# aanna0701/face-recognition-pytorch

Hardware: AMD Instinct MI355X
Metric: train imgs/sec IR-50-layout ResNet50 + ArcFace/PartialFC head, 112x112 (higher is better)
Workload: dtype bf16

## Files before the change

face-recognition-pytorch_amd/frhip/csrc/igemm_halo.h:

```cpp
#pragma once
#include <type_traits>
#include "igemm_nt.h"

#ifndef FRHIP_ABL
#define FRHIP_ABL 0
#endif

namespace frhip {

struct HaloGeom {
    int H, W, C;
    int M, Nout, Ktot;
    int sign;
    uint32_t a_bytes, b_bytes;
    const float* xf_scale;
    const float* xf_shift;
    void* xf_out;
    FastDiv d_hw, d_w;
};

template <typename T, int WM, int WN, int MT, int HBUFS>
struct HaloTile {
    static constexpr int WAVES = WM * WN, THREADS = 64 * WAVES;
    static constexpr int WROWS = MT * 16, BM = WM * WROWS, BN = WN * 64;
    static constexpr int BKE = NT_ROWB / (int)sizeof(T);
    static constexpr int MAXW = 56;
    static constexpr int HROWS = ((BM + 2 * MAXW + 2 + 7) / 8) * 8;
    static constexpr int ZROW = HROWS * NT_ROWB;
    static constexpr int HALO_BYTES = ZROW + NT_ROWB;
    static constexpr int WBUF_BYTES = BN * NT_ROWB;
    static constexpr int DUMP_OFF = HBUFS * HALO_BYTES;
    static constexpr int W_OFF = DUMP_OFF + 1024;
    static constexpr int WRING = 3;
    static constexpr int B_PIECES = (BN / 8 + WAVES - 1) / WAVES;
    static constexpr int ITER_PIECES = B_PIECES + (HBUFS == 2 ? 1 : 0);
    template <typename TS> static constexpr int stage_pitch() { return 64 * (int)sizeof(TS) + 16; }
    template <typename TS> static constexpr int lds_bytes() {
        constexpr int loop = W_OFF + WRING * WBUF_BYTES;
        constexpr int epi = WAVES * WROWS * stage_pitch<TS>();
        return loop > epi ? loop : epi;
    }
};

template <typename T, int WM, int WN, int MT, int HBUFS, bool XF = false>
struct HaloMainloop {
    static_assert(!XF || (HBUFS == 1 && std::is_same<T, bf16_t>::value), "operand transform: single-buffer bf16 tile only");
    typedef HaloTile<T, WM, WN, MT, HBUFS> Tile;
    typedef typename Mma<T>::Frag Frag;
    static constexpr int BM = Tile::BM, BN = Tile::BN, BKE = Tile::BKE;

    f32x4_t acc[4][MT];

    __device__ __forceinline__ void run(const HaloGeom& g, const void* __restrict__ a_ptr,
                                        const void* __restrict__ b_ptr, char* smem, int mtile, int ntile) {
        const int lane = lane_id(), wave = wave_id();
        const int wm = wave / WN, wn = wave % WN;
        const __amdgpu_buffer_rsrc_t ra = make_rsrc(a_ptr, g.a_bytes);
        const __amdgpu_buffer_rsrc_t rb = make_rsrc(b_ptr, g.b_bytes);
        const int m0 = mtile * BM;
        const int hrows = BM + 2 * g.W + 2;
        const int npieces = (hrows + 7) >> 3;
        const int p_lo = m0 - g.W - 1;
        const int sub = lane >> 3;
        const uint32_t chunk_bytes = (uint32_t)(((lane & 7) ^ sub) * 16);
        const int nchunks = g.C / BKE;

        const uint32_t row0_off = (uint32_t)((p_lo + sub) * g.C) * (uint32_t)sizeof(T) + chunk_bytes;
        auto halo_piece = [&](int hb, int piece, int c0) {
            const uint32_t off = row0_off + (uint32_t)(piece * 8 * g.C + c0) * (uint32_t)sizeof(T);
            glds16(ra, smem + hb * Tile::HALO_BYTES + piece * 1024, off);
        };
        auto xform_chunk = [&](int c0) {
            if constexpr (XF) {
                const int lc = (lane & 7) ^ sub;
                float sc[8], sh[8];
#pragma unroll
                for (int e = 0; e < 8; ++e) { sc[e] = g.xf_scale[c0 + 8 * lc + e]; sh[e] = g.xf_shift[c0 + 8 * lc + e]; }
                const bool emit = g.xf_out != nullptr && ntile == 0;
                for (int piece = wave; piece < npieces; piece += Tile::WAVES) {
                    const int p = p_lo + piece * 8 + sub;
                    if (p >= 0 && p < g.M) {
                        bf16x8_t* a = reinterpret_cast<bf16x8_t*>(smem + piece * 1024 + lane * 16);
                        bf16x8_t v = *a;
#pragma unroll
                        for (int e = 0; e < 8; ++e) { const float o = (float)v[e] * sc[e] + sh[e]; v[e] = (bf16_t)fmaxf(o, 0.f); }
                        *a = v;
                        if (emit && p >= m0 && p < m0 + BM)
                            *reinterpret_cast<bf16x8_t*>(reinterpret_cast<bf16_t*>(g.xf_out) + (size_t)p * g.C + c0 + 8 * lc) = v;
                    }
                }
                asm volatile("s_waitcnt lgkmcnt(0)" ::: "memory");
            }
        };
        uint32_t brow_off[Tile::B_PIECES];
#pragma unroll
        for (int j = 0; j < Tile::B_PIECES; ++j) {
            const int piece = wave * Tile::B_PIECES + j;
            const int n = ntile * BN + piece * 8 + sub;
            brow_off[j] = (piece * 8 < BN && n < g.Nout) ? (uint32_t)n * (uint32_t)g.Ktot * (uint32_t)sizeof(T) + chunk_bytes
                                                         : OOB_OFFSET;
        }
        auto weights = [&](int wit) {
            const int ch = wit / 9, tap = wit - ch * 9;
            const bool live = ch < nchunks;
            const uint32_t kb = (uint32_t)(tap * g.C + ch * BKE) * (uint32_t)sizeof(T);
            char* wb = smem + Tile::W_OFF + (wit % Tile::WRING) * Tile::WBUF_BYTES;
#pragma unroll
            for (int j = 0; j < Tile::B_PIECES; ++j) {
                const int piece = wave * Tile::B_PIECES + j;
                const bool in_tile = piece * 8 < BN;
                glds16(rb, in_tile ? wb + piece * 1024 : smem + Tile::DUMP_OFF,
                       (live && in_tile && brow_off[j] != OOB_OFFSET) ? brow_off[j] + kb : OOB_OFFSET);
            }
        };

        const int fi = lane & 15, fg = lane >> 4;
        static_assert(Tile::HALO_BYTES < 65536, "packed fragment offsets");
        uint32_t xa[9][(MT + 1) / 2];
        {
            const int HW = g.H * g.W;
            uint32_t tt[9];
#pragma unroll
// ... 61 lines not shown
                for (int nt = 0; nt < 4; ++nt) {
                    if constexpr (FRHIP_ABL & 2) { Frag fa = wf[SET][nt], fb = xf[SET][mt]; asm volatile("" :: "v"(fa), "v"(fb)); }
                    else Mma<T>::run(wf[SET][nt], xf[SET][mt], acc[nt][mt]);
                }
        };
        auto mfma_set_first = [&](auto set_c) {
            constexpr int SET = decltype(set_c)::value;
#pragma unroll
            for (int mt = 0; mt < MT; ++mt)
#pragma unroll
                for (int nt = 0; nt < 4; ++nt) {
                    f32x4_t z = f32x4_t{0.f, 0.f, 0.f, 0.f};
                    if constexpr (FRHIP_ABL & 2) { Frag fa = wf[SET][nt], fb = xf[SET][mt]; asm volatile("" :: "v"(fa), "v"(fb)); }
                    else Mma<T>::run(wf[SET][nt], xf[SET][mt], z);
                    acc[nt][mt] = z;
                }
        };
        auto interleave = [&]() {
            constexpr int NREAD = (4 + MT) * (int)(sizeof(Frag) / 16), NMFMA = 4 * MT * (sizeof(T) == 2 ? 1 : (sizeof(T) == 1 ? 2 : 4));
            constexpr int PER = NMFMA / NREAD > 0 ? NMFMA / NREAD : 1;
#pragma unroll
            for (int i = 0; i < NREAD; ++i) {
                __builtin_amdgcn_sched_group_barrier(0x008, PER, 0);
                __builtin_amdgcn_sched_group_barrier(0x100, 1, 0);
            }
        };
        typedef std::integral_constant<int, 0> I0;
        typedef std::integral_constant<int, 1> I1;

        if (threadIdx.x < 8 * HBUFS) {
            const int hbz = threadIdx.x >> 3;
            *reinterpret_cast<f32x4_t*>(smem + hbz * Tile::HALO_BYTES + Tile::ZROW + (threadIdx.x & 7) * 16) = f32x4_t{0.f, 0.f, 0.f, 0.f};
        }
        for (int piece = wave; piece < npieces; piece += Tile::WAVES) halo_piece(0, piece, 0);
        weights(0);
        weights(1);
        asm volatile("s_waitcnt vmcnt(0)" ::: "memory");
        xform_chunk(0);
        __syncthreads();
        load_frags(I0{}, I0{}, I0{}, I0{}, I0{});

        auto chunk_body = [&](auto hb_c, int ch) {
            constexpr int HB = decltype(hb_c)::value;
            constexpr int HBN = HBUFS == 2 ? (HB ^ 1) : 0;
            const int c0 = ch * BKE;
            const int it0 = ch * 9;
            auto tap_body = [&](auto tap_c) {
                constexpr int TAP = decltype(tap_c)::value;
                if constexpr (!(FRHIP_ABL & 8)) {
                    weights(it0 + TAP + 2);
                    if (HBUFS == 2) {
                        const int piece = TAP * Tile::WAVES + wave;
                        if (TAP < 8 && ch + 1 < nchunks && piece < npieces) halo_piece(HBN, piece, c0 + BKE);
                        else glds16(ra, smem + Tile::DUMP_OFF, OOB_OFFSET);
                    }
                }
                load_frags(I1{}, I1{}, hb_c, std::integral_constant<int, TAP % Tile::WRING>{}, tap_c);
                if (TAP == 0 && ch == 0) mfma_set_first(I0{});
                else mfma_set(I0{});
                interleave();
                if constexpr (FRHIP_ABL & 8) asm volatile("s_waitcnt vmcnt(0)" ::: "memory");
                else if constexpr (Tile::ITER_PIECES == 1) asm volatile("s_waitcnt vmcnt(1)" ::: "memory");
                else if constexpr (Tile::ITER_PIECES == 2) asm volatile("s_waitcnt vmcnt(2)" ::: "memory");
                else if constexpr (Tile::ITER_PIECES == 3) asm volatile("s_waitcnt vmcnt(3)" ::: "memory");
                else if constexpr (Tile::ITER_PIECES == 4) asm volatile("s_waitcnt vmcnt(4)" ::: "memory");
                else asm volatile("s_waitcnt vmcnt(5)" ::: "memory");
                static_assert(Tile::ITER_PIECES <= 5, "add a vmcnt case");
                if constexpr (!(FRHIP_ABL & 1)) __builtin_amdgcn_s_barrier();
                if constexpr (TAP < 8)
                    load_frags(I0{}, I0{}, hb_c, std::integral_constant<int, (TAP + 1) % Tile::WRING>{}, std::integral_constant<int, (TAP + 1) % 9>{});
                else
                    load_frags(I0{}, I0{}, std::integral_constant<int, HBN>{}, I0{}, I0{});
                mfma_set(I1{});
                interleave();
            };
            tap_body(std::integral_constant<int, 0>{}); tap_body(std::integral_constant<int, 1>{});
            tap_body(std::integral_constant<int, 2>{}); tap_body(std::integral_constant<int, 3>{});
            tap_body(std::integral_constant<int, 4>{}); tap_body(std::integral_constant<int, 5>{});
            tap_body(std::integral_constant<int, 6>{}); tap_body(std::integral_constant<int, 7>{});
            tap_body(std::integral_constant<int, 8>{});
            if (HBUFS == 1 && ch + 1 < nchunks) {
                asm volatile("s_waitcnt lgkmcnt(0)" ::: "memory");
                __builtin_amdgcn_s_barrier();
                for (int piece = wave; piece < npieces; piece += Tile::WAVES) halo_piece(0, piece, c0 + BKE);
                asm volatile("s_waitcnt vmcnt(0)" ::: "memory");
                xform_chunk(c0 + BKE);
                __builtin_amdgcn_s_barrier();
                load_frags(I0{}, I0{}, I0{}, I0{}, I0{});
            }
        };
        static_assert(HBUFS == 1 || Tile::HROWS / 8 <= 8 * Tile::WAVES, "eight halo slices must cover the halo");
        for (int ch = 0; ch < nchunks; ch += HBUFS) {
            chunk_body(std::integral_constant<int, 0>{}, ch);
            if (HBUFS == 2 && ch + 1 < nchunks) chunk_body(std::integral_constant<int, HBUFS - 1>{}, ch + 1);
        }
        asm volatile("s_waitcnt vmcnt(0)" ::: "memory");
    }

    template <typename TS>
    __device__ __forceinline__ char* stage_out(char* smem) {
        constexpr int P = Tile::template stage_pitch<TS>();
        const int lane = lane_id();
        const int fi = lane & 15, fg = lane >> 4;
        char* mine = smem + wave_id() * Tile::WROWS * P;
        __syncthreads();
#pragma unroll
        for (int nt = 0; nt < 4; ++nt)
#pragma unroll
            for (int mt = 0; mt < MT; ++mt) {
                char* p = mine + (mt * 16 + fi) * P + (nt * 16 + 4 * fg) * (int)sizeof(TS);
                if constexpr (sizeof(TS) == 4) {
                    *reinterpret_cast<f32x4_t*>(p) = acc[nt][mt];
                } else {
                    bf16x4_t v;
#pragma unroll
                    for (int e = 0; e < 4; ++e) v[e] = (bf16_t)acc[nt][mt][e];
                    *reinterpret_cast<bf16x4_t*>(p) = v;
                }
            }
// ... 7 lines not shown
```

face-recognition-pytorch_amd/frhip/csrc/igemm_halo.hip:

```cpp
#include "igemm_halo.h"
#include "igemm_halo_wide.h"
#include "frhip.h"

namespace frhip {

#ifndef FRHIP_CLOCK_STAMP
#define FRHIP_CLOCK_STAMP 0
#endif
#if FRHIP_CLOCK_STAMP
__device__ unsigned long long g_clock_stamps[2 * 8192];
#endif

template <typename T, int WM, int WN, int MT, int HBUFS, bool XF = false, bool LEAN = false>
__device__ __forceinline__ void halo_body(const HaloGeom& g, const void* __restrict__ a, const void* __restrict__ b,
                                          void* __restrict__ out, const void* __restrict__ res, float* __restrict__ stats,
                                          const EpiBnRed& br, char* smem, int mtile, int ntile) {
    typedef HaloTile<T, WM, WN, MT, HBUFS> Tile;
    HaloMainloop<T, WM, WN, MT, HBUFS, XF> ml;
#if FRHIP_CLOCK_STAMP
    const unsigned long long t0 = __builtin_amdgcn_s_memtime(), r0 = __builtin_amdgcn_s_memrealtime();
#endif
    ml.run(g, a, b, smem, mtile, ntile);
#if FRHIP_CLOCK_STAMP
    if (threadIdx.x == 0) {
        const unsigned long long t1 = __builtin_amdgcn_s_memtime(), r1 = __builtin_amdgcn_s_memrealtime();
        g_clock_stamps[2 * (blockIdx.x & 8191)] = t1 - t0;
        g_clock_stamps[2 * (blockIdx.x & 8191) + 1] = r1 - r0;
    }
#endif
    if constexpr (FRHIP_ABL & 16) {
        if (g.M >= 0) {
#pragma unroll
            for (int i = 0; i < 4; ++i)
#pragma unroll
                for (int j = 0; j < MT; ++j) asm volatile("" :: "v"(ml.acc[i][j]));
            return;
        }
    }
    const int wave = wave_id();
    const int wm = wave / WN, wn = wave % WN;
    const int m0 = mtile * Tile::BM + wm * Tile::WROWS, n0 = ntile * Tile::BN + wn * 64;
    EpiOperands<T, Tile::WROWS> eo;
    if constexpr (LEAN) {
        eo.fetch_fast(res, stats ? br.y : nullptr, g.M, g.Nout, m0, n0);
        const char* mine = ml.template stage_out<T>(smem);
        nt_epilogue_store_fast<T, WM, WN, Tile::WROWS, Tile::THREADS, Tile::BN>(mine, Tile::template stage_pitch<T>(), smem, g.M, g.Nout,
                                                                                out, res != nullptr, stats, br, eo, mtile, ntile);
    } else {
        eo.fetch(res, (stats || br.gelu_bwd) ? br.y : nullptr, g.M, g.Nout, m0, n0, br.res_h, br.res_w, &br.map);
        const char* mine = ml.template stage_out<T>(smem);
        nt_epilogue_store<T, WM, WN, Tile::WROWS, Tile::THREADS, Tile::BN>(mine, Tile::template stage_pitch<T>(), smem, g.M, g.Nout,
                                                                           out, res != nullptr, stats, br, eo, mtile, ntile, m0, n0);
    }
}

template <typename T, int WM, int WN, int MT, int HBUFS, bool XF = false, bool LEAN = false>
__global__ __launch_bounds__(64 * WM * WN, 2) void halo_kernel(HaloGeom g, const void* __restrict__ a,
                                                                         const void* __restrict__ b, void* __restrict__ out,
                                                                         const void* __restrict__ res, float* __restrict__ stats,
                                                                         EpiBnRed br, int mtiles, int ntiles) {
    extern __shared__ __attribute__((aligned(16))) char smem[];
    const uint32_t lin = xcd_remap(blockIdx.x, gridDim.x);
    const int ntile = (int)(lin % (uint32_t)ntiles), mtile = (int)(lin / (uint32_t)ntiles);
    halo_body<T, WM, WN, MT, HBUFS, XF, LEAN>(g, a, b, out, res, stats, br, smem, mtile, ntile);
}

template <bool LEAN>
__global__ __launch_bounds__(256, 2) void halo_wide_kernel(HaloGeom g, const void* __restrict__ a, const void* __restrict__ b,
                                                           void* __restrict__ out, const void* __restrict__ res,
                                                           float* __restrict__ stats, EpiBnRed br, int mtiles, int ntiles) {
    typedef HaloWideTile Tile;
    typedef bf16_t T;
    extern __shared__ __attribute__((aligned(16))) char smem[];
    const uint32_t lin = xcd_remap(blockIdx.x, gridDim.x);
    const int ntile = (int)(lin % (uint32_t)ntiles), mtile = (int)(lin / (uint32_t)ntiles);
    const int m_tile0 = mtile * Tile::BM;
    HaloWideMainloop ml;
#if FRHIP_CLOCK_STAMP
    const unsigned long long t0 = __builtin_amdgcn_s_memtime(), r0 = __builtin_amdgcn_s_memrealtime();
#endif
    ml.run(g, a, b, smem, m_tile0, ntile);
#if FRHIP_CLOCK_STAMP
    if (threadIdx.x == 0) {
        const unsigned long long t1 = __builtin_amdgcn_s_memtime(), r1 = __builtin_amdgcn_s_memrealtime();
        g_clock_stamps[2 * (blockIdx.x & 8191)] = t1 - t0;
        g_clock_stamps[2 * (blockIdx.x & 8191) + 1] = r1 - r0;
    }
#endif
    const int m0 = m_tile0 + wave_id() * Tile::WROWS;
#pragma unroll
    for (int half = 0; half < 2; ++half) {
        const int n0 = ntile * Tile::BN + half * 64;
        EpiOperands<T, Tile::WROWS> eo;
        if constexpr (LEAN) {
            eo.fetch_fast(res, stats ? br.y : nullptr, g.M, g.Nout, m0, n0);
            const char* mine = ml.stage_out(smem, half);
            nt_epilogue_store_fast<T, 4, 1, Tile::WROWS, Tile::THREADS, 64>(mine, Tile::stage_pitch, smem, g.M, g.Nout, out, res != nullptr,
                                                                            stats, br, eo, mtile, ntile * 2 + half);
        } else {
            eo.fetch(res, (stats || br.gelu_bwd) ? br.y : nullptr, g.M, g.Nout, m0, n0, br.res_h, br.res_w, &br.map);
            const char* mine = ml.stage_out(smem, half);
            nt_epilogue_store<T, 4, 1, Tile::WROWS, Tile::THREADS, 64>(mine, Tile::stage_pitch, smem, g.M, g.Nout, out, res != nullptr,
                                                                       stats, br, eo, mtile, ntile * 2 + half, m0, n0);
        }
    }
}

int g_epi_lean = 1;

static int halo_wide_launch(const HaloGeom& g, const void* a, const void* b, void* out, const void* res, float* stats,
                            const EpiBnRed& br, hipStream_t stream) {
    typedef HaloWideTile Tile;
    const int mtiles = (g.M + Tile::BM - 1) / Tile::BM, ntiles = (g.Nout + Tile::BN - 1) / Tile::BN;
    const bool lean = g_epi_lean && epi_lean_ok(true, g.M, g.Nout, Tile::BM, Tile::BN, br);
    auto kern = lean ? halo_wide_kernel<true> : halo_wide_kernel<false>;
    if (set_dynamic_lds(reinterpret_cast<const void*>(kern), Tile::LDS, "igemm_halo")) return FRHIP_ELAUNCH;
    hipLaunchKernelGGL(kern, dim3(mtiles * ntiles), dim3(Tile::THREADS), Tile::LDS, stream, g, a, b, out, res, stats, br, mtiles, ntiles);
    return check_launch("igemm_halo_wide");
}

template <typename T, int WM, int WN, int MT, int HBUFS, bool XF = false>
static int halo_launch(const HaloGeom& g, const void* a, const void* b, void* out, const void* res, float* stats,
                       const EpiBnRed& br, hipStream_t stream) {
    typedef HaloTile<T, WM, WN, MT, HBUFS> Tile;
    const int mtiles = (g.M + Tile::BM - 1) / Tile::BM, ntiles = (g.Nout + Tile::BN - 1) / Tile::BN;
    const int lds = Tile::template lds_bytes<T>();
    constexpr bool HAS_LEAN = sizeof(T) == 2 && WM == 4 && WN == 1 && MT == 4 && HBUFS == 1;
    bool lean = false;
    if constexpr (HAS_LEAN) lean = g_epi_lean && epi_lean_ok(true, g.M, g.Nout, Tile::BM, Tile::BN, br);
    auto kern = halo_kernel<T, WM, WN, MT, HBUFS, XF, false>;
    if constexpr (HAS_LEAN) { if (lean) kern = halo_kernel<T, WM, WN, MT, HBUFS, XF, true>; }
    if (set_dynamic_lds(reinterpret_cast<const void*>(kern), lds, "igemm_halo")) return FRHIP_ELAUNCH;
    hipLaunchKernelGGL(kern, dim3(mtiles * ntiles), dim3(Tile::THREADS), lds, stream, g, a, b, out, res, stats, br, mtiles, ntiles);
    return check_launch("igemm_halo");
}

static int g_halo_enabled = 1;

bool halo_applicable(int dtype, int h, int w, int c, int k, int r, int s, int stride, int pad) {
    const int bke = NT_ROWB / (dtype == FRHIP_DT_BF16 ? 2 : 4);
    return g_halo_enabled && r == 3 && s == 3 && stride == 1 && pad == 1 && w <= 56 && (c % bke) == 0 && (k % 8) == 0 &&
           (dtype == FRHIP_DT_BF16 || dtype == FRHIP_DT_F32);
}

static int g_halo_wide_dirs = 2;
static int halo_config(int dtype, int c, int k);
static int halo_config_w(int dtype, int w, int c, int k, int sign) {
    if ((g_halo_wide_dirs & (sign > 0 ? 1 : 2)) && dtype == FRHIP_DT_BF16 && w <= HaloWideTile::MAXW &&
        (k % 128) == 0 && (c % 64) == 0 && c >= 128 && (g_halo_enabled & 3) == 1)
        return 3;
    return halo_config(dtype, c, k);
}
static int halo_config(int dtype, int c, int k) {
    const int es = dtype == FRHIP_DT_BF16 ? 2 : 4;
    const int nchunks = c / (NT_ROWB / es);
    const bool narrow = (k % 128) != 0;
    if (dtype == FRHIP_DT_BF16) {
        const int mode = g_halo_enabled & 3;
        const bool two_per_cu = mode == 2 || (mode != 3 && nchunks <= 8);
        if (two_per_cu || narrow) return (nchunks == 1 || two_per_cu) ? 0 : 1;
        return 2;
    }
    return narrow ? 1 : 2;
}

bool halo_lean_applies(int dtype, int n, int h, int w, int c, int k, int sign) {
    if (!g_epi_lean || dtype != FRHIP_DT_BF16) return false;
    const long long M = 1LL * n * h * w;
    const int cfg = halo_config_w(dtype, w, c, k, sign) == 3 ? 3 : halo_config(dtype, c, k);
    const int bn = cfg == 3 ? HaloWideTile::BN : 64;
    if (cfg != 3 && cfg != 0) return false;
    return M % 256 == 0 && k % bn == 0 && M * k * 2 < 0x7fffffffLL;
}

int halo_stat_rows(int, int m, int, int, int, int) { return (m + 255) / 256; }

bool halo_xf_applicable(int dtype, int h, int w, int c, int k, int r, int s, int stride, int pad) {
    return dtype == FRHIP_DT_BF16 && halo_applicable(dtype, h, w, c, k, r, s, stride, pad) && halo_config(dtype, c, k) == 0;
}

int halo_run(int dtype, const void* a, const void* b, void* out, const void* res, float* stats, const EpiBnRed& br,
             int n, int h, int w, int c, int k, int sign, hipStream_t stream, const float* xf_scale, const float* xf_shift, void* xf_out) {
    const int es = dtype == FRHIP_DT_BF16 ? 2 : 4;
    const long long ab = 1LL * n * h * w * c * es, bb = 1LL * k * 9 * c * es;
    if (ab > 0x7fffffffLL || bb > 0x7fffffffLL) { set_error("igemm_halo: tensor exceeds the 2 GiB buffer window"); return FRHIP_EINVAL; }
    HaloGeom g;
    g.H = h; g.W = w; g.C = c; g.M = n * h * w; g.Nout = k; g.Ktot = 9 * c; g.sign = sign;
    g.a_bytes = (uint32_t)ab; g.b_bytes = (uint32_t)bb;
    g.xf_scale = xf_scale; g.xf_shift = xf_shift; g.xf_out = xf_out;
    g.d_hw = make_fastdiv((uint32_t)(h * w)); g.d_w = make_fastdiv((uint32_t)w);
    const int cfg = halo_config(dtype, c, k);
    if (xf_scale) {
        if (dtype != FRHIP_DT_BF16 || cfg != 0) { set_error("igemm_halo: operand transform not available for this shape"); return FRHIP_EINVAL; }
        return halo_launch<bf16_t, 4, 1, 4, 1, true>(g, a, b, out, res, stats, br, stream);
    }
    if (halo_config_w(dtype, w, c, k, sign) == 3) return halo_wide_launch(g, a, b, out, res, stats, br, stream);
    if (dtype == FRHIP_DT_BF16) {
        if (cfg == 0) return halo_launch<bf16_t, 4, 1, 4, 1>(g, a, b, out, res, stats, br, stream);
        if (cfg == 1) return halo_launch<bf16_t, 8, 1, 2, 2>(g, a, b, out, res, stats, br, stream);
        return halo_launch<bf16_t, 4, 2, 4, 2>(g, a, b, out, res, stats, br, stream);
    }
    if (cfg == 1) return halo_launch<float, 8, 1, 2, 2>(g, a, b, out, res, stats, br, stream);
    return halo_launch<float, 4, 2, 4, 2>(g, a, b, out, res, stats, br, stream);
}

}

#if FRHIP_CLOCK_STAMP
extern "C" int frhip_dbg_clock_read(unsigned long long* host, int pairs) {
    if (pairs > 8192) pairs = 8192;
    return hipMemcpyFromSymbol(host, HIP_SYMBOL(frhip::g_clock_stamps), sizeof(unsigned long long) * 2 * pairs) == hipSuccess ? 0 : -1;
}
#endif

extern "C" int frhip_set_epi_lean(int enabled) {
    const int old = frhip::g_epi_lean;
    if (enabled >= 0) frhip::g_epi_lean = enabled != 0;
    return old;
}

extern "C" int frhip_set_halo_wide_dirs(int dirs) {
    const int old = frhip::g_halo_wide_dirs;
    if (dirs >= 0) frhip::g_halo_wide_dirs = dirs & 3;
    return old;
}

// ... 6 lines not shown
```

face-recognition-pytorch_amd/frhip/csrc/igemm_nt.hip:

```cpp
#include "igemm_nt.h"
#include "frhip.h"

namespace frhip {

bool halo_applicable(int dtype, int h, int w, int c, int k, int r, int s, int stride, int pad);
int halo_stat_rows(int dtype, int m, int w, int c, int k, int sign);
bool halo_xf_applicable(int dtype, int h, int w, int c, int k, int r, int s, int stride, int pad);
bool halo_lean_applies(int dtype, int n, int h, int w, int c, int k, int sign);
int halo_run(int dtype, const void* a, const void* b, void* out, const void* res, float* stats, const EpiBnRed& br,
             int n, int h, int w, int c, int k, int sign, hipStream_t stream, const float* xf_scale = nullptr,
             const float* xf_shift = nullptr, void* xf_out = nullptr);

enum { EPI_STORE = 0, EPI_ATOMIC = 1, EPI_SLAB = 2, EPI_LEAN = 3 };
extern int g_epi_lean;

template <typename T, int WM, int WN, int MT, int EPI>
__device__ __forceinline__ void nt_tile(const NtGeom& g, const void* __restrict__ a, const void* __restrict__ b, void* __restrict__ out,
                                        const void* __restrict__ res, float* __restrict__ stats, const EpiBnRed& br, int ntiles,
                                        uint32_t t, uint32_t total, char* smem) {
    typedef NtTile<T, WM, WN, MT> Tile;
    constexpr int WROWS = Tile::WROWS, THREADS = Tile::THREADS;
    const uint32_t lin = xcd_remap(t, total);
    const int ntile = (int)(lin % (uint32_t)ntiles), mtile = (int)(lin / (uint32_t)ntiles);
    const int ks_begin = blockIdx.y * g.ksteps_per_split;
// ... 187 lines not shown
                              int n, int h, int wd, int c, int k, int r, int s, int stride, int pad,
                              hipStream_t stream) {
    NtGeom g;
    const int ho = (h + 2 * pad - r) / stride + 1, wo = (wd + 2 * pad - s) / stride + 1;
    int rc = fill_geom(g, dtype, n, h, wd, c, ho, wo, k, r, s, stride, pad, 0, "frhip_conv_fwd");
    if (rc) return rc;
    if (halo_applicable(dtype, h, wd, c, k, r, s, stride, pad))
        return halo_run(dtype, x, w, y, nullptr, stats_partial, NO_BNRED, n, h, wd, c, k, +1, stream);
    return nt_dispatch(dtype, g, x, w, y, nullptr, stats_partial, NO_BNRED, 1, false, stream);
}

extern "C" int frhip_conv_fwd_affine(int dtype, const void* x, const void* w, void* y, const float* scale, const float* shift, int relu,
                                     const void* residual, int n, int h, int wd, int c, int k, int r, int s, int stride, int pad,
                                     hipStream_t stream) {
    if (!scale || !shift) { set_error("frhip_conv_fwd_affine: scale and shift are required"); return FRHIP_EINVAL; }
    NtGeom g;
    const int ho = (h + 2 * pad - r) / stride + 1, wo = (wd + 2 * pad - s) / stride + 1;
    int rc = fill_geom(g, dtype, n, h, wd, c, ho, wo, k, r, s, stride, pad, 0, "frhip_conv_fwd_affine");
    if (rc) return rc;
    if (halo_applicable(dtype, h, wd, c, k, r, s, stride, pad) && halo_lean_applies(dtype, n, h, wd, c, k, +1)) {
        EpiBnRed br = NO_BNRED;
        br.aff_scale = scale; br.aff_shift = shift; br.aff_relu = relu;
        return halo_run(dtype, x, w, y, residual, nullptr, br, n, h, wd, c, k, +1, stream);
    }
    rc = frhip_conv_fwd(dtype, x, w, y, nullptr, n, h, wd, c, k, r, s, stride, pad, stream);
    if (rc) return rc;
    return frhip_bn_apply(dtype, y, scale, shift, residual, nullptr, nullptr, relu, y, n * ho * wo, k, stream);
}

extern "C" int frhip_conv_bnrelu_fusable(int dtype, int h, int wd, int c, int k, int r, int s, int stride, int pad) {
    return halo_xf_applicable(dtype, h, wd, c, k, r, s, stride, pad) ? 1 : 0;
}

extern "C" int frhip_conv_fwd_bnrelu(int dtype, const void* x, const float* in_scale, const float* in_shift, const void* w, void* y,
                                     float* stats_partial, void* act_out, int n, int h, int wd, int c, int k, int r, int s, int stride,
                                     int pad, hipStream_t stream) {
    if (!in_scale || !in_shift || !halo_xf_applicable(dtype, h, wd, c, k, r, s, stride, pad)) {
        set_error("frhip_conv_fwd_bnrelu: not fusable for this shape (ask frhip_conv_bnrelu_fusable first)");
        return FRHIP_EINVAL;
    }
    return halo_run(dtype, x, w, y, nullptr, stats_partial, NO_BNRED, n, h, wd, c, k, +1, stream, in_scale, in_shift, act_out);
}

static int dgrad_run(int dtype, const void* dy, const void* wt, void* dx, const void* residual, float* stats,
                     const EpiBnRed& br, int n, int h, int wd, int c, int k, int r, int s, int stride, int pad,
                     hipStream_t stream, const char* who) {
    NtGeom g;
    const int ho = (h + 2 * pad - r) / stride + 1, wo = (wd + 2 * pad - s) / stride + 1;
    int rc = fill_geom(g, dtype, n, ho, wo, k, h, wd, c, r, s, stride, pad, 1, who);
    if (rc) return rc;
    if (halo_applicable(dtype, h, wd, k, c, r, s, stride, pad))
        return halo_run(dtype, dy, wt, dx, residual, stats, br, n, h, wd, k, c, -1, stream);
    if (dgrad_by_parity(g)) {
        float* st = stats;
        for (int cls = 0; cls < 4; ++cls) {
            NtGeom gc; EpiBnRed bc = br;
            if (parity_class(g, dtype, cls >> 1, cls & 1, gc, bc.map) == 0) continue;
            rc = nt_dispatch(dtype, gc, dy, wt, dx, residual, st, bc, 1, false, stream);
            if (rc) return rc;
            if (st) st += (size_t)((gc.M + nt_block_rows(dtype, gc) - 1) / nt_block_rows(dtype, gc)) * 2 * gc.Nout;
        }
        return FRHIP_OK;
    }
    return nt_dispatch(dtype, g, dy, wt, dx, residual, stats, br, 1, false, stream);
}

// ... 133 lines not shown
```

face-recognition-pytorch_amd/frhip/ops.py:

```python
import math
import weakref

import ctypes

import torch

from . import _abi
from ._abi import DT_BF16, DT_F32, check, lib

_DT = {torch.bfloat16: DT_BF16, torch.float32: DT_F32}


def dt_of(t):
    return _DT[t.dtype]


def epv(dtype):
    return 8 if dtype == torch.bfloat16 else 4


def _s():
    return torch._C._cuda_getCurrentRawStream(torch.cuda.current_device())


# ... 62 lines not shown
            assert rowscale.dtype == torch.float32 and rowscale.is_contiguous() and rowscale.numel() * rows_per == n * h * wd
        if tuple(y_bn.shape) != tuple(x_shape) or y_bn.dtype != dy.dtype:
            raise ValueError("conv_dgrad(bnred): y_bn must have the shape and dtype of dx")
        rows = lib().frhip_dgrad_stat_rows(dt_of(dy), n, h, wd, c, k, r, s, stride, pad)
        part = torch.empty((rows, 2, c), dtype=torch.float32, device=dy.device)
    if rowscale is not None:
        check(lib().frhip_conv_dgrad_fused_rs(dt_of(dy), _p(dy), _p(wt), _p(dx), _p(residual), residual_stride, _p(y_bn), _p(st.mean),
                                              _p(st.invstd), _p(st.scale) if relu_mask else None, _p(st.shift) if relu_mask else None,
                                              _p(rowscale), rows_per, keep_scale, _p(part), n, h, wd, c, k, r, s, stride, pad, _s()),
              "frhip_conv_dgrad_fused_rs")
        return dx, part
    check(lib().frhip_conv_dgrad_fused(dt_of(dy), _p(dy), _p(wt), _p(dx), _p(residual), residual_stride, _p(y_bn),
                                       _p(st.mean) if st else None, _p(st.invstd) if st else None,
                                       _p(st.scale) if relu_mask else None, _p(st.shift) if relu_mask else None, _p(part),
                                       n, h, wd, c, k, r, s, stride, pad, _s()), "frhip_conv_dgrad_fused")
    return dx if bnred is None else (dx, part)


_FUSABLE = {}


def conv_bnrelu_fusable(x, w, stride, pad):
    n, h, wd, c = x.shape
    k, r, s, _ = w.shape
    key = (x.dtype, n, h, wd, c, k, r, s, stride, pad)
    hit = _FUSABLE.get(key)
    if hit is None:
        hit = _FUSABLE[key] = x.dtype in _DT and \
            bool(lib().frhip_conv_bnrelu_fusable(dt_of(x), h, wd, c, k, r, s, stride, pad)) and \
            bool(lib().frhip_conv_wgrad_bnrelu_fusable(dt_of(x), n, h, wd, c, k, r, s, stride, pad))
    return hit


def conv_fwd_bnrelu(x, st, w, stride, pad, want_stats=True, act_out=None):
    n, h, wd, c = x.shape
    k, r, s, c2 = w.shape
    assert c == c2 and x.dtype == w.dtype
    ho, wo = conv_out_hw(h, wd, r, s, stride, pad)
    y = torch.empty((n, ho, wo, k), dtype=x.dtype, device=x.device)
    part = None
    if want_stats:
        rows = lib().frhip_conv_stat_rows(dt_of(x), n * ho * wo, k, h, wd, c, r, s, stride, pad)
        part = torch.empty((rows, 2, k), dtype=torch.float32, device=x.device)
    check(lib().frhip_conv_fwd_bnrelu(dt_of(x), _p(x), _p(st.scale), _p(st.shift), _p(w), _p(y), _p(part), _p(act_out), n, h, wd, c, k,
                                      r, s, stride, pad, _s()), "frhip_conv_fwd_bnrelu")
    return y, part


_WORKSPACES = {}
WORKSPACE_BYTES = 160 << 20


def workspace(device):
    key = (torch.device(device).index, _s())
    ws = _WORKSPACES.get(key)
    if ws is None:
        ws = _WORKSPACES[key] = torch.empty(WORKSPACE_BYTES // 4, dtype=torch.float32, device=device)
    return ws


def conv_wgrad(dy, x, dw, r, s, stride, pad, splits=0):
    n, h, wd, c = x.shape
    k = dy.shape[3]
    ws = workspace(x.device)
    check(lib().frhip_conv_wgrad(dt_of(x), _p(dy), _p(x), _p(dw), n, h, wd, c, k, r, s, stride, pad, splits,
                                 _p(ws), ws.numel() * 4, _s()), "frhip_conv_wgrad")
# ... 1013 lines not shown
```

face-recognition-pytorch_amd/nets/_backbone.py:

```python
import os

import torch
import torch.distributed as dist
import torch.nn as nn

from frhip import ops
from frhip.optim import DEFERRED_SIDE, run_deferred_side

_OVERLAP_WGRAD = os.environ.get("FRHIP_OVERLAP_WGRAD", "1") == "1"
_STEM_FUSED_REDUCE = True
_FUSE_BN1 = True
_EVAL_FOLD = True
_WGRAD_LATE_MAXC = 64
_DTYPES = {"bf16": torch.bfloat16, "bfloat16": torch.bfloat16, "fp32": torch.float32, "float32": torch.float32}


def compute_dtype(conf):
    name = getattr(conf, "frhip_dtype", None) or os.environ.get("FRHIP_DTYPE", "bf16")
    return _DTYPES[str(name).lower()]


class _Conv(nn.Module):

    def __init__(self, cin, cout, k, stride, bias=False, pad=None):
# ... 378 lines not shown

    def take(self, x):
        if self._of is x:
            return self._x8
        return ops.quant_fp8(x)


def basic_block_forward(blk, xin, dt, training, save, wprep=None, q8=None):
    cin, planes = blk.conv1.cin, blk.conv2.cout
    if not training and not save and q8 is None and _EVAL_FOLD:
        w1, _ = _operands(blk.conv1, dt, wprep)
        w2, _ = _operands(blk.conv2, dt, wprep)
        a1 = ops.conv_fwd_affine(xin, w1, bn_forward_state(blk.bn1, None, 0, False), 1, 1, relu=True)
        res = xin
        if blk.downsample is not None:
            dconv, dbn = blk.downsample[0], blk.downsample[1]
            wd, _ = _operands(dconv, dt, wprep)
            res = ops.conv_fwd_affine(xin, wd, bn_forward_state(dbn, None, 0, False), dconv.stride, 0)
        out = ops.conv_fwd_affine(a1, w2, bn_forward_state(blk.bn2, None, 0, False), blk.stride, 1, residual=res)
        return out, None
    f1 = q8 is not None and dt == torch.bfloat16 and Fp8Ctx.eligible(cin)
    fo = q8 is not None and dt == torch.bfloat16 and Fp8Ctx.eligible(planes)
    w1, w1t = _operands(blk.conv1, dt, wprep)
    x8 = q8.take(xin) if f1 else None
    if f1:
        y1, p1 = ops.conv_fwd_fp8(x8, *q8.packs[blk.conv1], 1, 1, want_stats=training)
    else:
        y1, p1 = ops.conv_fwd(xin, w1, 1, 1, want_stats=training)
    st1 = bn_forward_state(blk.bn1, p1, y1.numel() // y1.shape[3], training)
    w2, w2t = _operands(blk.conv2, dt, wprep)
    if f1:
        a1, a18 = ops.bn_apply_q8(y1, st1, relu=True)
        y2, p2 = ops.conv_fwd_fp8(a18, *q8.packs[blk.conv2], blk.stride, 1, want_stats=training)
    elif _FUSE_BN1 and ops.conv_bnrelu_fusable(y1, w2, blk.stride, 1):
        a1 = torch.empty_like(y1) if save else None
        y2, p2 = ops.conv_fwd_bnrelu(y1, st1, w2, blk.stride, 1, want_stats=training, act_out=a1)
    else:
        a1 = ops.bn_apply(y1, st1, relu=True)
        y2, p2 = ops.conv_fwd(a1, w2, blk.stride, 1, want_stats=training)
    st2 = bn_forward_state(blk.bn2, p2, y2.numel() // y2.shape[3], training)
    yd = std = wdt = None
    res, res_st = xin, None
    if blk.downsample is not None:
        dconv, dbn = blk.downsample[0], blk.downsample[1]
        wd, wdt = _operands(dconv, dt, wprep)
        if f1:
            yd, pd = ops.conv_fwd_fp8(x8, *q8.packs[dconv], dconv.stride, 0, want_stats=training)
        else:
            yd, pd = ops.conv_fwd(xin, wd, dconv.stride, 0, want_stats=training)
        std = bn_forward_state(dbn, pd, yd.numel() // yd.shape[3], training)
        res, res_st = yd, std
    if fo:
        out, out8 = ops.bn_apply_q8(y2, st2, res=res, res_st=res_st)
        q8.put(out, out8)
    else:
        out = ops.bn_apply(y2, st2, res=res, res_st=res_st)
    s = None
    if save:
        s = Saved()
        s.x, s.y1, s.st1, s.a1, s.y2, s.st2, s.yd, s.std = xin, y1, st1, a1, y2, st2, yd, std
        s.w1t, s.w2t, s.wdt = w1t, w2t, wdt
    return out, s


def basic_block_backward(blk, s, dout, dt, bc, part2=None, next_bn=None):
    G = bc.G
    dy2 = ops.bn_backward(dout, s.y2, s.st2, blk.bn2.weight.data, G(blk.bn2.weight), G(blk.bn2.bias), part=part2)
# ... 128 lines not shown
```

include/frhip.h:

```cpp
#ifndef FRHIP_H
#define FRHIP_H
#include <stddef.h>
#include <stdint.h>

#ifdef __cplusplus
extern "C" {
#endif

#ifndef FRHIP_STREAM_T
#define FRHIP_STREAM_T
#ifdef __HIP_PLATFORM_AMD__
#include <hip/hip_runtime_api.h>
typedef hipStream_t frhip_stream_t;
#else
typedef void* frhip_stream_t;
#endif
#endif

#define FRHIP_OK 0
#define FRHIP_EINVAL (-1)
#define FRHIP_ELAUNCH (-2)
#define FRHIP_DT_BF16 0
#define FRHIP_DT_F32 1

// ... 141 lines not shown
                         int d, const frhip_margin_t* margin, const float* rowmax, const float* rowsum, float gscale,
                         const float* upstream, void* dt, int ldt, void* dtt, int ldtt, frhip_stream_t stream);

typedef struct { float s, eps; const float* m_ang; const float* m_add; } frhip_margin_rows_t;
int frhip_adaface_margins(const float* norms, int n, double m, double h, double t_alpha, double eps, int update, float* batch_mean,
                          float* batch_std, float* m_ang, float* m_add, frhip_stream_t stream);
int frhip_head_fwd_rows(int dtype, const void* ehat, const void* what, const int* labels, int n, int classes,
                        int d, const frhip_margin_rows_t* margin, float* part_max, float* part_sum, float* ztarget,
                        float* rowmax, float* rowsum, frhip_stream_t stream);
int frhip_head_bwd_dt_rows(int dtype, const void* ehat, const void* what, const int* labels, int n, int classes,
                           int d, const frhip_margin_rows_t* margin, const float* rowmax, const float* rowsum, float gscale,
                           const float* upstream, void* dt, int ldt, void* dtt, int ldtt, frhip_stream_t stream);

int frhip_head_sub_max(void);
int frhip_head_fwd_sub(int dtype, const void* ehat, const void* what, const int* labels, int n, int classes, int d,
                       int subcenters, const frhip_margin_t* margin, float* part_max, float* part_sum, float* ztarget,
                       int* tsub, float* rowmax, float* rowsum, frhip_stream_t stream);
int frhip_head_fwd_sub_rows(int dtype, const void* ehat, const void* what, const int* labels, int n, int classes, int d,
                            int subcenters, const frhip_margin_rows_t* margin, float* part_max, float* part_sum,
                            float* ztarget, int* tsub, float* rowmax, float* rowsum, frhip_stream_t stream);
int frhip_head_bwd_dt_sub(int dtype, const void* ehat, const void* what, const int* labels, int n, int classes, int d,
                          int subcenters, const frhip_margin_t* margin, const float* rowmax, const float* rowsum,
                          float gscale, const float* upstream, void* dt, int ldt, int ldp, void* dtt, int ldtt,
                          frhip_stream_t stream);
int frhip_head_bwd_dt_sub_rows(int dtype, const void* ehat, const void* what, const int* labels, int n, int classes, int d,
                               int subcenters, const frhip_margin_rows_t* margin, const float* rowmax, const float* rowsum,
                               float gscale, const float* upstream, void* dt, int ldt, int ldp, void* dtt, int ldtt,
                               frhip_stream_t stream);

int frhip_conv_bnrelu_fusable(int dtype, int h, int wd, int c, int k, int r, int s, int stride, int pad);
int frhip_conv_fwd_bnrelu(int dtype, const void* x, const float* in_scale, const float* in_shift, const void* w, void* y,
                          float* stats_partial, void* act_out, int n, int h, int wd, int c, int k, int r, int s, int stride,
                          int pad, frhip_stream_t stream);
int frhip_conv_wgrad_bnrelu_fusable(int dtype, int n, int h, int w, int c, int k, int r, int s, int stride, int pad);
int frhip_conv_wgrad_bnrelu(int dtype, const void* dy, const void* x, const float* in_scale, const float* in_shift,
                            float* dw, int n, int h, int w, int c, int k, int r, int s, int stride, int pad, int splits,
                            float* workspace, size_t workspace_bytes, frhip_stream_t stream);

int frhip_quant_fp8_weights(const float* w, void* w8, float* scale, int k, int rowlen, frhip_stream_t stream);
typedef struct { const float* w; void* w8; float* scale; int32_t k, rowlen, row_begin, pad_; } frhip_q8w;
int frhip_quant_fp8_weights_multi(const frhip_q8w* table, int ntensors, int nrows, frhip_stream_t stream);
int frhip_fp8_saturation(int op);
int frhip_quant_fp8(int dtype, const void* x, void* x8, size_t n, float inv_scale, frhip_stream_t stream);
int frhip_bn_apply_q8(int dtype, const void* y, const float* scale, const float* shift, const void* res,
                      const float* res_scale, const float* res_shift, int relu, void* out, void* out8, float inv_q,
                      int rows, int c, frhip_stream_t stream);
int frhip_conv_fwd_fp8(const void* x8, const void* w8, const float* wscale, float act_scale, void* y,
                       float* stats_partial, int n, int h, int wd, int c, int k, int r, int s, int stride, int pad,
                       frhip_stream_t stream);
int frhip_fp8_stat_rows(int m, int k);
int frhip_fp8_conv_stat_rows(int m, int k, int h, int w, int c, int r, int s, int stride, int pad);
int frhip_set_fp8_halo(int enabled);
int frhip_linear_fwd_fp8(const void* a8, const void* w8, const float* wscale, float act_scale, const float* bias,
                         void* out, float* stats_partial, int m, int n, int k, frhip_stream_t stream);

typedef struct frhip_cpb_block {
    const void* coords;
    const void* index;
    const void* w0;
    const void* b0;
    const void* w2;
    const void* logit_scale;
    void* bias;
    void* scale;
    const void* dbias;
    const void* dscale;
// ... 113 lines not shown
```

Baseline: 23000.

## Stage BN coefficients in LDS, spread activation emission across N-tiles, gate fusion by K

The fused BN+ReLU operand transform in the halo conv now preloads per-channel scale and shift into extra LDS once per block instead of re-reading them from global memory each chunk. The transform loop is unrolled with unconditional LDS reads, and the activation write-back goes through buffer stores. That write-back is now spread round-robin across N-tiles (chunk ch is emitted by tile ch mod ntiles) instead of always by tile 0. A new 'preferred' predicate limits the fused path to K<=512 and C<=512, so larger layers fall back to the unfused path. This costs extra LDS per block, which may lower occupancy.

```diff
diff --git a/face-recognition-pytorch_amd/frhip/csrc/igemm_halo.h b/face-recognition-pytorch_amd/frhip/csrc/igemm_halo.h
--- a/face-recognition-pytorch_amd/frhip/csrc/igemm_halo.h
+++ b/face-recognition-pytorch_amd/frhip/csrc/igemm_halo.h
@@ -34,6 +34,7 @@
     static constexpr int WRING = 3;
     static constexpr int B_PIECES = (BN / 8 + WAVES - 1) / WAVES;
     static constexpr int ITER_PIECES = B_PIECES + (HBUFS == 2 ? 1 : 0);
+    static constexpr int XF_MAX_C = 512, XF_COEF_BYTES = 2 * XF_MAX_C * 4;
     template <typename TS> static constexpr int stage_pitch() { return 64 * (int)sizeof(TS) + 16; }
     template <typename TS> static constexpr int lds_bytes() {
         constexpr int loop = W_OFF + WRING * WBUF_BYTES;
@@ -52,7 +53,7 @@
     f32x4_t acc[4][MT];
 
     __device__ __forceinline__ void run(const HaloGeom& g, const void* __restrict__ a_ptr,
-                                        const void* __restrict__ b_ptr, char* smem, int mtile, int ntile) {
+                                        const void* __restrict__ b_ptr, char* smem, int mtile, int ntile, int ntiles = 1) {
         const int lane = lane_id(), wave = wave_id();
         const int wm = wave / WN, wn = wave % WN;
         const __amdgpu_buffer_rsrc_t ra = make_rsrc(a_ptr, g.a_bytes);
@@ -70,24 +71,47 @@
             const uint32_t off = row0_off + (uint32_t)(piece * 8 * g.C + c0) * (uint32_t)sizeof(T);
             glds16(ra, smem + hb * Tile::HALO_BYTES + piece * 1024, off);
         };
-        auto xform_chunk = [&](int c0) {
+        constexpr int XF_NPW = (Tile::HROWS / 8 + Tile::WAVES - 1) / Tile::WAVES;
+        constexpr int XF_NSURE = ((BM + 4 + 7) / 8) / Tile::WAVES;
+        static_assert(!XF || ((XF_NPW - 1) * Tile::WAVES + Tile::WAVES) * 1024 <= Tile::W_OFF, "unconditional piece reads stay inside the tile");
+        const int xf_lc = (lane & 7) ^ sub;
+        f32x4_t xsc[2], xsh[2];
+        auto xform_coeffs = [&](int c0) {
             if constexpr (XF) {
-                const int lc = (lane & 7) ^ sub;
-                float sc[8], sh[8];
-#pragma unroll
-                for (int e = 0; e < 8; ++e) { sc[e] = g.xf_scale[c0 + 8 * lc + e]; sh[e] = g.xf_shift[c0 + 8 * lc + e]; }
-                const bool emit = g.xf_out != nullptr && ntile == 0;
-                for (int piece = wave; piece < npieces; piece += Tile::WAVES) {
-                    const int p = p_lo + piece * 8 + sub;
-                    if (p >= 0 && p < g.M) {
-                        bf16x8_t* a = reinterpret_cast<bf16x8_t*>(smem + piece * 1024 + lane * 16);
-                        bf16x8_t v = *a;
-#pragma unroll
-                        for (int e = 0; e < 8; ++e) { const float o = (float)v[e] * sc[e] + sh[e]; v[e] = (bf16_t)fmaxf(o, 0.f); }
-                        *a = v;
-                        if (emit && p >= m0 && p < m0 + BM)
-                            *reinterpret_cast<bf16x8_t*>(reinterpret_cast<bf16_t*>(g.xf_out) + (size_t)p * g.C + c0 + 8 * lc) = v;
+                const f32x4_t* cs = reinterpret_cast<const f32x4_t*>(smem + Tile::template lds_bytes<T>() + (c0 + 8 * xf_lc) * 4);
+                const f32x4_t* ch = reinterpret_cast<const f32x4_t*>(smem + Tile::template lds_bytes<T>() + (g.C + c0 + 8 * xf_lc) * 4);
+                xsc[0] = cs[0]; xsc[1] = cs[1]; xsh[0] = ch[0]; xsh[1] = ch[1];
+            }
+        };
+        auto xform_chunk = [&](int c0, bool emit) {
+            if constexpr (XF) {
+                const __amdgpu_buffer_rsrc_t ro = make_rsrc(g.xf_out, g.a_bytes);
+                const int nw = (npieces - wave + Tile::WAVES - 1) / Tile::WAVES;
+                char* mine = smem + wave * 1024 + lane * 16;
+                const int r0 = wave * 8 + sub;
+                const uint32_t off0 = row0_off + (uint32_t)(wave * 8 * g.C + c0) * (uint32_t)sizeof(T);
+                const uint32_t ostep = (uint32_t)(Tile::WAVES * 8 * g.C) * (uint32_t)sizeof(T);
+                bf16x8_t v[XF_NPW];
+#pragma unroll
+                for (int i = 0; i < XF_NPW; ++i) v[i] = *reinterpret_cast<const bf16x8_t*>(mine + i * Tile::WAVES * 1024);
+                auto one = [&](int i) {
+                    const int r = r0 + i * Tile::WAVES * 8;
+                    bf16x8_t o;
+#pragma unroll
+                    for (int e = 0; e < 8; ++e) { const float f = (float)v[i][e] * xsc[e >> 2][e & 3] + xsh[e >> 2][e & 3]; o[e] = (bf16_t)fmaxf(f, 0.f); }
+                    const bool in_tensor = (uint32_t)(p_lo + r) < (uint32_t)g.M;
+                    *reinterpret_cast<bf16x8_t*>(in_tensor ? mine + i * Tile::WAVES * 1024 : smem + Tile::DUMP_OFF + lane * 16) = o;
+                    if (emit) {
+                        const bool own = (uint32_t)(r - g.W - 1) < (uint32_t)BM;
+                        __builtin_amdgcn_raw_buffer_store_b128(__builtin_bit_cast(u32x4_t, o), ro, (int)(own ? off0 + (uint32_t)i * ostep : OOB_OFFSET), 0, 0);
                     }
+                };
+#pragma unroll
+                for (int i = 0; i < XF_NSURE; ++i) one(i);
+#pragma unroll
+                for (int i = XF_NSURE; i < XF_NPW; ++i) {
+                    asm volatile("" : "+v"(v[i]));
+                    if (i < nw) one(i);
                 }
                 asm volatile("s_waitcnt lgkmcnt(0)" ::: "memory");
             }
@@ -215,11 +239,19 @@
             const int hbz = threadIdx.x >> 3;
             *reinterpret_cast<f32x4_t*>(smem + hbz * Tile::HALO_BYTES + Tile::ZROW + (threadIdx.x & 7) * 16) = f32x4_t{0.f, 0.f, 0.f, 0.f};
         }
+        int emit_ch = ntile;
+        if constexpr (XF) {
+            float* cf = reinterpret_cast<float*>(smem + Tile::template lds_bytes<T>());
+            for (int i = threadIdx.x * 4; i < 2 * g.C; i += Tile::THREADS * 4)
+                *reinterpret_cast<f32x4_t*>(cf + i) = *reinterpret_cast<const f32x4_t*>((i < g.C ? g.xf_scale : g.xf_shift - g.C) + i);
+            if (g.xf_out == nullptr) emit_ch = nchunks;
+        }
         for (int piece = wave; piece < npieces; piece += Tile::WAVES) halo_piece(0, piece, 0);
         weights(0);
         weights(1);
+        if constexpr (XF) { __syncthreads(); xform_coeffs(0); }
         asm volatile("s_waitcnt vmcnt(0)" ::: "memory");
-        xform_chunk(0);
+        if constexpr (XF) { xform_chunk(0, emit_ch == 0); if (emit_ch == 0) emit_ch += ntiles; }
         __syncthreads();
         load_frags(I0{}, I0{}, I0{}, I0{}, I0{});
 
@@ -265,9 +297,10 @@
             if (HBUFS == 1 && ch + 1 < nchunks) {
                 asm volatile("s_waitcnt lgkmcnt(0)" ::: "memory");
                 __builtin_amdgcn_s_barrier();
+                if constexpr (XF) xform_coeffs(c0 + BKE);
                 for (int piece = wave; piece < npieces; piece += Tile::WAVES) halo_piece(0, piece, c0 + BKE);
                 asm volatile("s_waitcnt vmcnt(0)" ::: "memory");
-                xform_chunk(c0 + BKE);
+                if constexpr (XF) { const bool emit = emit_ch == ch + 1; xform_chunk(c0 + BKE, emit); if (emit) emit_ch += ntiles; }
                 __builtin_amdgcn_s_barrier();
                 load_frags(I0{}, I0{}, I0{}, I0{}, I0{});
             }
diff --git a/face-recognition-pytorch_amd/frhip/csrc/igemm_halo.hip b/face-recognition-pytorch_amd/frhip/csrc/igemm_halo.hip
--- a/face-recognition-pytorch_amd/frhip/csrc/igemm_halo.hip
+++ b/face-recognition-pytorch_amd/frhip/csrc/igemm_halo.hip
@@ -14,13 +14,14 @@
 template <typename T, int WM, int WN, int MT, int HBUFS, bool XF = false, bool LEAN = false>
 __device__ __forceinline__ void halo_body(const HaloGeom& g, const void* __restrict__ a, const void* __restrict__ b,
                                           void* __restrict__ out, const void* __restrict__ res, float* __restrict__ stats,
-                                          const EpiBnRed& br, char* smem, int mtile, int ntile) {
+                                          const EpiBnRed& br, char* smem, int mtile, int ntile, int ntiles) {
     typedef HaloTile<T, WM, WN, MT, HBUFS> Tile;
     HaloMainloop<T, WM, WN, MT, HBUFS, XF> ml;
 #if FRHIP_CLOCK_STAMP
     const unsigned long long t0 = __builtin_amdgcn_s_memtime(), r0 = __builtin_amdgcn_s_memrealtime();
 #endif
-    ml.run(g, a, b, smem, mtile, ntile);
+    if constexpr (XF) ml.run(g, a, b, smem, mtile, ntile, ntiles);
+    else ml.run(g, a, b, smem, mtile, ntile);
 #if FRHIP_CLOCK_STAMP
     if (threadIdx.x == 0) {
         const unsigned long long t1 = __builtin_amdgcn_s_memtime(), r1 = __builtin_amdgcn_s_memrealtime();
@@ -62,7 +63,7 @@
     extern __shared__ __attribute__((aligned(16))) char smem[];
     const uint32_t lin = xcd_remap(blockIdx.x, gridDim.x);
     const int ntile = (int)(lin % (uint32_t)ntiles), mtile = (int)(lin / (uint32_t)ntiles);
-    halo_body<T, WM, WN, MT, HBUFS, XF, LEAN>(g, a, b, out, res, stats, br, smem, mtile, ntile);
+    halo_body<T, WM, WN, MT, HBUFS, XF, LEAN>(g, a, b, out, res, stats, br, smem, mtile, ntile, ntiles);
 }
 
 template <bool LEAN>
@@ -124,7 +125,7 @@
                        const EpiBnRed& br, hipStream_t stream) {
     typedef HaloTile<T, WM, WN, MT, HBUFS> Tile;
     const int mtiles = (g.M + Tile::BM - 1) / Tile::BM, ntiles = (g.Nout + Tile::BN - 1) / Tile::BN;
-    const int lds = Tile::template lds_bytes<T>();
+    const int lds = Tile::template lds_bytes<T>() + (XF ? Tile::XF_COEF_BYTES : 0);
     constexpr bool HAS_LEAN = sizeof(T) == 2 && WM == 4 && WN == 1 && MT == 4 && HBUFS == 1;
     bool lean = false;
     if constexpr (HAS_LEAN) lean = g_epi_lean && epi_lean_ok(true, g.M, g.Nout, Tile::BM, Tile::BN, br);
@@ -176,7 +177,8 @@
 int halo_stat_rows(int, int m, int, int, int, int) { return (m + 255) / 256; }
 
 bool halo_xf_applicable(int dtype, int h, int w, int c, int k, int r, int s, int stride, int pad) {
-    return dtype == FRHIP_DT_BF16 && halo_applicable(dtype, h, w, c, k, r, s, stride, pad) && halo_config(dtype, c, k) == 0;
+    return dtype == FRHIP_DT_BF16 && halo_applicable(dtype, h, w, c, k, r, s, stride, pad) && halo_config(dtype, c, k) == 0 &&
+           c <= HaloTile<bf16_t, 4, 1, 4, 1>::XF_MAX_C;
 }
 
 int halo_run(int dtype, const void* a, const void* b, void* out, const void* res, float* stats, const EpiBnRed& br,
@@ -191,7 +193,7 @@
     g.d_hw = make_fastdiv((uint32_t)(h * w)); g.d_w = make_fastdiv((uint32_t)w);
     const int cfg = halo_config(dtype, c, k);
     if (xf_scale) {
-        if (dtype != FRHIP_DT_BF16 || cfg != 0) { set_error("igemm_halo: operand transform not available for this shape"); return FRHIP_EINVAL; }
+        if (dtype != FRHIP_DT_BF16 || cfg != 0 || c > HaloTile<bf16_t, 4, 1, 4, 1>::XF_MAX_C) { set_error("igemm_halo: operand transform not available for this shape"); return FRHIP_EINVAL; }
         return halo_launch<bf16_t, 4, 1, 4, 1, true>(g, a, b, out, res, stats, br, stream);
     }
     if (halo_config_w(dtype, w, c, k, sign) == 3) return halo_wide_launch(g, a, b, out, res, stats, br, stream);
diff --git a/face-recognition-pytorch_amd/frhip/csrc/igemm_nt.hip b/face-recognition-pytorch_amd/frhip/csrc/igemm_nt.hip
--- a/face-recognition-pytorch_amd/frhip/csrc/igemm_nt.hip
+++ b/face-recognition-pytorch_amd/frhip/csrc/igemm_nt.hip
@@ -243,6 +243,14 @@
     return halo_xf_applicable(dtype, h, wd, c, k, r, s, stride, pad) ? 1 : 0;
 }
 
+#ifndef FRHIP_XF_PREFER_MAX_K
+#define FRHIP_XF_PREFER_MAX_K 512
+#endif
+extern "C" int frhip_conv_bnrelu_preferred(int dtype, int n, int h, int wd, int c, int k, int r, int s, int stride, int pad) {
+    (void)n;
+    return halo_xf_applicable(dtype, h, wd, c, k, r, s, stride, pad) && k <= FRHIP_XF_PREFER_MAX_K ? 1 : 0;
+}
+
 extern "C" int frhip_conv_fwd_bnrelu(int dtype, const void* x, const float* in_scale, const float* in_shift, const void* w, void* y,
                                      float* stats_partial, void* act_out, int n, int h, int wd, int c, int k, int r, int s, int stride,
                                      int pad, hipStream_t stream) {
diff --git a/face-recognition-pytorch_amd/frhip/ops.py b/face-recognition-pytorch_amd/frhip/ops.py
--- a/face-recognition-pytorch_amd/frhip/ops.py
+++ b/face-recognition-pytorch_amd/frhip/ops.py
@@ -118,6 +118,13 @@
     return hit
 
 
+def conv_bnrelu_preferred(x, w, stride, pad):
+    n, h, wd, c = x.shape
+    k, r, s, _ = w.shape
+    return conv_bnrelu_fusable(x, w, stride, pad) and \
+        bool(lib().frhip_conv_bnrelu_preferred(dt_of(x), n, h, wd, c, k, r, s, stride, pad))
+
+
 def conv_fwd_bnrelu(x, st, w, stride, pad, want_stats=True, act_out=None):
     n, h, wd, c = x.shape
     k, r, s, c2 = w.shape
diff --git a/face-recognition-pytorch_amd/nets/_backbone.py b/face-recognition-pytorch_amd/nets/_backbone.py
--- a/face-recognition-pytorch_amd/nets/_backbone.py
+++ b/face-recognition-pytorch_amd/nets/_backbone.py
@@ -434,7 +434,7 @@
     if f1:
         a1, a18 = ops.bn_apply_q8(y1, st1, relu=True)
         y2, p2 = ops.conv_fwd_fp8(a18, *q8.packs[blk.conv2], blk.stride, 1, want_stats=training)
-    elif _FUSE_BN1 and ops.conv_bnrelu_fusable(y1, w2, blk.stride, 1):
+    elif _FUSE_BN1 and ops.conv_bnrelu_preferred(y1, w2, blk.stride, 1):
         a1 = torch.empty_like(y1) if save else None
         y2, p2 = ops.conv_fwd_bnrelu(y1, st1, w2, blk.stride, 1, want_stats=training, act_out=a1)
     else:
diff --git a/include/frhip.h b/include/frhip.h
--- a/include/frhip.h
+++ b/include/frhip.h
@@ -197,6 +197,7 @@
 int frhip_conv_fwd_bnrelu(int dtype, const void* x, const float* in_scale, const float* in_shift, const void* w, void* y,
                           float* stats_partial, void* act_out, int n, int h, int wd, int c, int k, int r, int s, int stride,
                           int pad, frhip_stream_t stream);
+int frhip_conv_bnrelu_preferred(int dtype, int n, int h, int wd, int c, int k, int r, int s, int stride, int pad);
 int frhip_conv_wgrad_bnrelu_fusable(int dtype, int n, int h, int w, int c, int k, int r, int s, int stride, int pad);
 int frhip_conv_wgrad_bnrelu(int dtype, const void* dy, const void* x, const float* in_scale, const float* in_shift,
                             float* dw, int n, int h, int w, int c, int k, int r, int s, int stride, int pad, int splits,
```

Result: no change. 23140 (median of 6 runs) (+0.6%).
